# moritzmeister/hops-examples

Measured on AMD Instinct MI355X. Metric: images/sec MNIST CNN + steps/sec Chicago-taxi DNN at 1/2/4/8 MI355X, higher is better.
Workload: dtype bf16; 1 GPU; model=MNIST CNN (experiment.mirrored model, 1394282 params), Adadelta(1.0), global_batch=32, per_gpu_batch=32, parallelism=dp1, engine=PersistentMnistStep, hipgraph=False, steps_per_execution=32, warmup_steps_run=5

## Files before the change

csrc/ops/bindings.cpp:

```cpp
#include <pybind11/pybind11.h>
#include <pybind11/stl.h>

#include <algorithm>
#include <memory>
#include <stdexcept>
#include <string>
#include <tuple>
#include <utility>
#include <vector>

#if defined(HOPSX_DEBUG) && HOPSX_DEBUG
#define HOPSX_DEBUG_BUILD 1
#else
#define HOPSX_DEBUG_BUILD 0
#endif

#include "ops_api.h"
extern "C" int hopsx_mnist_persist_occupancy(int dp);
extern "C" void hopsx_mnist_persist_reload_knobs();
extern "C" int hopsx_pad_cin(const float* w, long R, int C, int cp, float* out, void* out16, hipStream_t st);
extern "C" int hopsx_unpad_cin_add(float* gpad, long R, int C, int cp, float* tgt, hipStream_t st);

namespace py = pybind11;
extern "C" void hopsx_mlp_head_debug(void* p);
// ... 106 lines not shown
  if (!e) e = hopsx_det_set_##tag(on);
    HOPSX_DET_TUS(X)
#undef X
    return e;
  });
  m.attr("DEBUG") = HOPSX_DEBUG_BUILD;
  m.def("dbg_read", []() {
    static const std::pair<const char*, int (*)(unsigned*)> tus[] = {
#define X(tag) {#tag, hopsx_dbg_read_##tag},
        HOPSX_DBG_TUS(X)
#undef X
    };
    std::vector<std::tuple<std::string, unsigned, unsigned, unsigned, unsigned>> out;
    for (const auto& t : tus) {
      unsigned v[4] = {0u, 0u, 0u, 0u};
      const int e = t.second(v);
      if (e) throw std::runtime_error(std::string("hopsx dbg_read: hip error ") + std::to_string(e));
      if (v[0]) out.emplace_back(t.first, v[0], v[1], v[2], v[3]);
    }
    return out;
  });
  m.def("det_lost", []() {
    unsigned n = 0;
#define X(tag) n += hopsx_det_lost_##tag();
    HOPSX_DET_TUS(X)
#undef X
    return n;
  });
  m.def("mnist_persist", [](std::vector<uint64_t> p, std::vector<long> iv, std::vector<float> fv, u st) {
    return hopsx_mnist_persist(p.data(), (int)p.size(), iv.data(), (int)iv.size(), fv.data(), (int)fv.size(),
                               S(st));
  });
  def_arg_slots<false>(m, "mnist_persist", [](const ArgSlots& a, hipStream_t st) {
    return hopsx_mnist_persist(a.p.data(), (int)a.p.size(), a.iv.data(), (int)a.iv.size(), a.fv.data(),
                               (int)a.fv.size(), st);
  });
  m.def("mnist_eval", [](std::vector<uint64_t> p, std::vector<long> iv, std::vector<float> fv, u st) {
    return hopsx_mnist_eval(p.data(), (int)p.size(), iv.data(), (int)iv.size(), fv.data(), (int)fv.size(), S(st));
  });
  m.def("mnist_eval_tile", []() { return hopsx_mnist_eval_tile(); });
  m.def("taxi_eval", [](std::vector<uint64_t> p, std::vector<long> iv, u st) {
    return hopsx_taxi_eval(p.data(), (int)p.size(), iv.data(), (int)iv.size(), S(st));
  });
  m.def("taxi_eval_bins", []() { return hopsx_taxi_eval_bins(); });
  m.def("mnist_persist_reload_knobs", []() { hopsx_mnist_persist_reload_knobs(); });
  m.def("mnist_persist_occupancy", [](int dp) { return hopsx_mnist_persist_occupancy(dp); });
  m.def("pad_cin", [](u w, long R, int C, int cp, u out, u out16, u st) {
    return hopsx_pad_cin(P<float>(w), R, C, cp, P<float>(out), P<void>(out16), S(st));
  });
  m.def("unpad_cin_add", [](u g, long R, int C, int cp, u tgt, u st) {
    return hopsx_unpad_cin_add(P<float>(g), R, C, cp, P<float>(tgt), S(st));
  });
  m.def("mnist_persist_geom", []() {
    std::vector<long> g(23);
    hopsx_mnist_persist_geom(g.data());
    return g;
  });
  m.def("widedeep_step", [](std::vector<uint64_t> p, std::vector<long> iv, std::vector<float> fv, u st) {
    return hopsx_widedeep_step(p.data(), (int)p.size(), iv.data(), (int)iv.size(), fv.data(), (int)fv.size(),
                               S(st));
  });
  m.def("conv2d_fwd_pool_ok", [](std::vector<int> g, int act, int pk) { return hopsx_conv_fwd_pool_ok(g.data(), act, pk); });
  m.def("conv2d_fwd_pool", [](u x, u w, std::vector<int> g, u out, u am, u bias, int act, float p, u rng,
                              unsigned salt, int pk, u st) {
    return hopsx_conv2d_fwd_pool(P<void>(x), P<void>(w), g.data(), P<void>(out), P<void>(am), P<float>(bias), act, p,
                                 P<unsigned long long>(rng), salt, pk, S(st));
  });
  m.def("conv2d_fwd_pool_in_ok", [](std::vector<int> g0, std::vector<int> g, int act) {
    return hopsx_conv_fwd_pool_in_ok(g0.data(), g.data(), act);
  });
  m.def("conv2d_fwd_pool_in", [](u x0, float xscale, float xshift, u w0, u b0, int act0, std::vector<int> g0, u y1,
                                 u w, std::vector<int> g, u out, u am, u bias, int act, float p, u rng, unsigned salt,
                                 u st) {
    return hopsx_conv2d_fwd_pool_in(P<void>(x0), xscale, xshift, P<void>(w0), P<float>(b0), act0, g0.data(),
                                    P<void>(y1), P<void>(w), g.data(), P<void>(out), P<void>(am), P<float>(bias), act,
                                    p, P<unsigned long long>(rng), salt, S(st));
  });
  m.def("conv2d_dgrad_fused_wgrad_ok", [](std::vector<int> g, std::vector<int> g0) {
    return hopsx_conv_dgrad_fused_wgrad_ok(g.data(), g0.data());
  });
  m.def("conv2d_dgrad_fused_wgrad", [](u dy, u w, std::vector<int> g, u yprev, int act, u colsum, u y, int yact,
                                       std::vector<int> g0, u x0, float xscale, float xshift, u dw0, u st) {
    return hopsx_conv2d_dgrad_mfma_ex(P<void>(dy), P<void>(w), g.data(), nullptr, P<void>(yprev), act,
                                      P<float>(colsum), P<void>(y), yact, g0.data(), P<void>(x0), xscale, xshift,
                                      P<float>(dw0), S(st));
  });
  m.def("wgrad_debug_times", [](int n) {
    std::vector<unsigned long long> v((size_t)n);
    hopsx_wgrad_debug_times(v.data(), n);
    return v;
  });
  m.def("head_ce_ok", [](int C, int KD) { return hopsx_head_ce_ok(C, KD); });
  m.def("head_ce", [](int kind, u logits, int lf32, u target, int B, int C, int KD, float gs, u h, u w, u dw, u db,
                      u dh, u loss, u correct, u bias, u lout, float dp, u drng, unsigned dsalt, u st) {
    return hopsx_head_ce(kind, P<void>(logits), lf32, P<void>(target), B, C, KD, gs, P<void>(h), P<void>(w),
                         P<float>(dw), P<float>(db), P<void>(dh), P<float>(loss), P<int>(correct), P<float>(bias),
                         P<void>(lout), dp, P<unsigned long long>(drng), dsalt, S(st));
  });
  m.def("mlp_head_lds", [](int C, int N1) { return hopsx_mlp_head_lds(C, N1); });
  m.def("mlp_head_debug", [](u p) { hopsx_mlp_head_debug(P<void>(p)); });
  m.def("graph_upload", [](u exec, u st) {
    return (int)hipGraphUpload(reinterpret_cast<hipGraphExec_t>(exec), S(st));
  });
  m.def("mlp_head", [](u x, u w1, u b1, int act1, u y, u ws, u arrive, int B, int K, int N1, int kind, u target,
                       int C, float gs, u w2, u b2, u dw2, u db2, u dh, u loss, u correct, u lout, int lf32, float dp,
                       u drng, unsigned dsalt, u st) {
    return hopsx_mlp_head(P<void>(x), P<void>(w1), P<float>(b1), act1, P<void>(y), P<float>(ws), P<unsigned>(arrive),
// ... 208 lines not shown
```

csrc/ops/mnist_persist.hip:

```cpp
#include "common.h"
#include "mnist_cnn.h"
#include "optim_core.h"
#include "wg_prims.h"

namespace mnistp {
using namespace wgp;
using namespace mnist_cnn;

constexpr int B = 32;
constexpr int NCONV = C2 * 128 + C2 + C1 * 4 + C1;
constexpr int OFF_B2 = C2 * 128, OFF_W1 = OFF_B2 + C2, OFF_B1 = OFF_W1 + C1 * 4;
constexpr int SLICE = 64, NSLICE = (NCONV + SLICE - 1) / SLICE;
constexpr int NRED = 19;
constexpr int NKC = (NPOS + NRED - 1) / NRED;
constexpr int NQ = SLICE / 4;
constexpr int NHEAD = B;
constexpr int GRID = NPOS + NHEAD;
constexpr int PAY = 272;
constexpr int PAY_DH = 0, PAY_H = 128, PAY_DL = 256, PAY_LOSS = 268, PAY_COR = 269;
constexpr int FL_A = 0, FL_B = 256, FL_C = 512, FL_D = 768, FL_WORDS = 1024;
constexpr int FL_EPOCH = FL_WORDS - 2;
constexpr int D_F32 = OFF_B2 * 2;
constexpr int D_BYTES = D_F32 + (NCONV - OFF_B2) * 4;
constexpr int TGB_N = NHEAD * (HID / 2);
constexpr int TG_WORDS = 2 * 2 * TGB_N;
static_assert(FL_WORDS % 2 == 0 && TGB_N % 256 == 0, "granules are 8-B aligned; every thread owns TGB_N / 256");

constexpr int DHS = row_stride(HID), DCS = row_stride(4 * B);
static_assert(DHS == 136 && DCS == 136, "strides the kernel was tuned with");

constexpr int L_W1 = 0;
constexpr int L_W2 = L_W1 + HID * W1S * 2;
constexpr int L_CW1 = L_W2 + C2 * W2S * 2;
constexpr int L_CB1 = L_CW1 + C1 * 4 * 4;
constexpr int L_CB2 = L_CB1 + C1 * 4;
constexpr int L_XIN = L_CB2 + C2 * 4;
constexpr int L_C1 = L_XIN + B * 16 * 4;
constexpr int L_POOL = L_C1 + B * 9 * C1S * 2;
constexpr int L_AM = L_POOL + B * PLS * 2;
constexpr int L_DH = L_AM + B * C2;
constexpr int L_DC2 = L_DH + B * DHS * 2;
constexpr int L_STG = L_DC2 + C2 * DCS * 2;
constexpr int L_RED = L_STG + NCONV * 4;
constexpr int L_SL = L_RED + NRED * SLICE * 4;
constexpr int L_KEEP = L_SL + 3 * 64 * 4;
constexpr int LDS_BYTES = L_KEEP + B * C2;

constexpr int H_W2 = 0;
constexpr int H_B2 = H_W2 + 3 * NCLS * HID * 4;
constexpr int H_B1 = H_B2 + 3 * 16 * 4;
constexpr int H_RED = H_B1 + 3 * HID * 4;
constexpr int H_H = H_RED + 8 * HID * 4;
constexpr int H_LOG = H_H + HID * 4;
constexpr int H_PAY = H_LOG + 16 * 4;
constexpr int H_ALL = H_PAY + PAY * 4;
constexpr int H_END = H_ALL + NHEAD * PAY * 4;
constexpr int H_DHS = H_END;
static_assert(H_DHS + B * DHS * 2 <= LDS_BYTES, "head LDS map must fit the position map");

constexpr int XMAX = 8;
constexpr long XS_POOL = (long)NPOS * 4 * 64 * 16;
constexpr long XS_DHT = 8L * 64 * 16;
constexpr int NFC2 = NCLS * HID + HID + NCLS, NFC2P = 1424;
constexpr long XS_FC2 = NFC2P * 4;
constexpr long XS_CONV = (long)NSLICE * SLICE * 4;
constexpr long XO_POOL = 0, XO_DHT = XO_POOL + 2L * XMAX * XS_POOL, XO_FC2 = XO_DHT + 2L * XMAX * XS_DHT,
               XO_CONV = XO_FC2 + 2L * XMAX * XS_FC2, X_BYTES = XO_CONV + 2L * XMAX * XS_CONV;
constexpr int XF_POOL = 0, XF_H = XMAX * NPOS, XF_CONV = XF_H + XMAX, XF_WORDS = XF_CONV + XMAX * NSLICE;
static_assert(NFC2 <= NFC2P && NFC2P % 4 == 0 && X_BYTES < 0x7fffffffL, "exchange geometry");
static_assert(LDS_BYTES <= 160 * 1024, "one workgroup per CU: 160 KiB LDS");
static_assert(L_RED + NRED * SLICE * 4 <= L_SL && 2 * 32 * 5 * 4 <= NRED * SLICE * 4, "reduce scratch");
static_assert(SLICE * 4 % 128 == 0 && NCONV * 4 % 128 == 0, "a slice row is whole 128-byte lines of an aligned slabC row");
static_assert(OFF_B2 % SLICE == 0 && D_F32 % 128 == 0 && D_BYTES % 128 == 0, "no slice straddles the bf16 / fp32 parts of D");
static_assert(NSLICE * SLICE >= NCONV && NSLICE <= NPOS && SLICE == 64, "slice geometry: one wave updates a slice");
static_assert(NQ == 16 && NRED > 16 && NRED - 16 <= 3 && 5 * NKC <= 64 && 2 * NKC <= 32 && NRED * (NKC - 1) < NPOS,
              "gather geometry: at most 5 groups' flags per wave, one per lane; both items' rows in one pend mask");

struct Args {
  float* master;
// ... 196 lines not shown
      if (__builtin_amdgcn_readfirstlane(e) != 0u) {
        good = 0;
        break;
      }
      if ((spins & 15u) == 15u && wall_clock64() - t0 > tmo) {
        if (lane == 0) atomicCAS(err, 0u, code);
        good = 0;
        break;
      }
      __builtin_amdgcn_s_sleep(1);
    }
    if (lane == 0) *s_ok = good;
  }
  __syncthreads();
  const int v = *s_ok;
  return v != 0;
}
template <int N, class F>
__device__ __forceinline__ bool sweep_tags(const unsigned long long* g, int tid, unsigned epoch, unsigned* err,
                                        unsigned code, int* s_fail, long long tmo, F put) {
  unsigned pend = (1u << N) - 1u;
  unsigned long long x[N];
#pragma unroll
  for (int k = 0; k < N; ++k) x[k] = granule_load(g + tid + 256 * k);
  unsigned e = flag_load(err);
  const long long t0 = wall_clock64();
  for (unsigned spins = 0;; ++spins) {
#pragma unroll
    for (int k = 0; k < N; ++k)
      if (((pend >> k) & 1u) && (unsigned)(x[k] >> 32) == epoch) {
        put(tid + 256 * k, (unsigned)x[k]);
        pend &= ~(1u << k);
      }
    if (!__any(pend != 0u)) break;
    bool bad = __builtin_amdgcn_readfirstlane(e) != 0u;
    if (!bad && (spins & 15u) == 15u && wall_clock64() - t0 > tmo) {
      if ((threadIdx.x & 63) == 0) atomicCAS(err, 0u, code);
      bad = true;
    }
    if (bad) {
      if ((threadIdx.x & 63) == 0) *s_fail = 1;
      break;
    }
#pragma unroll
    for (int k = 0; k < N; ++k)
      if ((pend >> k) & 1u) x[k] = granule_load(g + tid + 256 * k);
    e = flag_load(err);
  }
  __syncthreads();
  const int f = *s_fail;
  return f == 0;
}

template <int NK, class L>
__device__ __forceinline__ void gather_rows(const unsigned* flag, bool mine, int shift, unsigned pend, unsigned epoch,
                                            unsigned* err, unsigned code, int* s_fail, long long tmo, L load) {
  const long long t0 = wall_clock64();
  for (unsigned spins = 0;; ++spins) {
    const unsigned e = flag_load(err);
    const unsigned f = mine ? flag_load(flag) : 0u;
    const unsigned long long here = __ballot(mine && f == epoch);
    const unsigned now = pend & (unsigned)(here >> shift);
#pragma unroll
    for (int k = 0; k < NK; ++k)
      if ((now >> k) & 1u) load(k);
    pend &= ~now;
    if (!__any(pend != 0u)) break;
    bool bad = __builtin_amdgcn_readfirstlane(e) != 0u;
    if (!bad && (spins & 15u) == 15u && wall_clock64() - t0 > tmo) {
      if ((threadIdx.x & 63) == 0) atomicCAS(err, 0u, code);
      bad = true;
    }
    if (bad) {
      if ((threadIdx.x & 63) == 0) *s_fail = 1;
      break;
    }
    __builtin_amdgcn_s_sleep(1);
  }
}

template <bool DP>
__device__ __forceinline__ void position_wg(const Args& a, unsigned char* smem, int* s_ok, const OptHP& hp,
                                            long long cur0, unsigned long long seed, unsigned long long ctr0,
                                            long long xs0, unsigned long long eb) {
  const int p = blockIdx.x, ph = p / PH, pw = p - ph * PH;
  const int tid = threadIdx.x, lane = tid & 63, w = tid >> 6, fr = lane & 15, fq = lane >> 4;
  const int tq = fr >> 2, tp = fr & 3;
  bf16_raw* W1 = (bf16_raw*)(smem + L_W1);
  bf16_raw* W2 = (bf16_raw*)(smem + L_W2);
  float* CW1 = (float*)(smem + L_CW1);
  float* CB1 = (float*)(smem + L_CB1);
  float* CB2 = (float*)(smem + L_CB2);
  float* XIN = (float*)(smem + L_XIN);
  bf16_raw* C1 = (bf16_raw*)(smem + L_C1);
  bf16_raw* POOL = (bf16_raw*)(smem + L_POOL);
  unsigned char* AM = smem + L_AM;
  bf16_raw* DH = (bf16_raw*)(smem + L_DH);
  bf16_raw* DC2 = (bf16_raw*)(smem + L_DC2);
  float* STG = (float*)(smem + L_STG);
  float* RED = (float*)(smem + L_RED);
  float* SLm = (float*)(smem + L_SL);
  float* SL1 = SLm + 64;
  float* SL2 = SLm + 128;

  float wm[2][4][4], g1[2][4][4], g2[2][4][4];
#pragma unroll
  for (int ii = 0; ii < 2; ++ii)
#pragma unroll
    for (int j = 0; j < 4; ++j)
#pragma unroll
      for (int r = 0; r < 4; ++r) {
        const int n = (2 * w + ii) * 16 + fq * 4 + r, co = j * 16 + fr;
        const long ai = a.off[4] + (long)n * KIN + p * C2 + co;
        wm[ii][j][r] = a.master[ai];
        g1[ii][j][r] = a.s1[ai];
        g2[ii][j][r] = a.s2[ai];
        W1[n * W1S + co] = f2bf_hw(wm[ii][j][r]);
      }
  auto put_conv = [&](int j, float v) {
    if (j < OFF_B2) W2[(j >> 7) * W2S + (j & 127)] = f2bf_hw(v);
    else if (j < OFF_W1) CB2[j - OFF_B2] = v;
    else if (j < OFF_B1) CW1[j - OFF_W1] = v;
    else CB1[j - OFF_B1] = v;
  };
  {
    constexpr int NJ = (NCONV + 255) / 256;
    float cv[NJ];
#pragma unroll
    for (int q = 0; q < NJ; ++q) {
      const int j = tid + 256 * q;
// ... 151 lines not shown
    stamp(a, s, 1);
    {
      f32x4 acc[2][2];
#pragma unroll
      for (int i = 0; i < 2; ++i)
#pragma unroll
        for (int jj = 0; jj < 2; ++jj) acc[i][jj] = (f32x4){0.f, 0.f, 0.f, 0.f};
      bf16x8 af[2][2], bfr[2][2];
#pragma unroll
      for (int kk = 0; kk < 2; ++kk) {
#pragma unroll
        for (int i = 0; i < 2; ++i) af[kk][i] = lds8(POOL + (i * 16 + fr) * PLS + kk * 32 + fq * 8);
#pragma unroll
        for (int jj = 0; jj < 2; ++jj) bfr[kk][jj] = lds8(W1 + ((2 * w + jj) * 16 + fr) * W1S + kk * 32 + fq * 8);
      }
      __builtin_amdgcn_sched_barrier(0);
#pragma unroll
      for (int kk = 0; kk < 2; ++kk)
#pragma unroll
        for (int i = 0; i < 2; ++i)
#pragma unroll
          for (int jj = 0; jj < 2; ++jj) acc[i][jj] = mma32(af[kk][i], bfr[kk][jj], acc[i][jj]);
#pragma unroll
      for (int i = 0; i < 2; ++i)
#pragma unroll
        for (int jj = 0; jj < 2; ++jj)
#pragma unroll
          for (int r = 0; r < 4; ++r) STG[(i * 16 + fq * 4 + r) * HID + (2 * w + jj) * 16 + fr] = acc[i][jj][r];
    }
    __syncthreads();
    {
      const auto R = rsrc(a.slabA + ((long)par * NPOS + p) * (B * HID));
      f32x4 v[4];
#pragma unroll
      for (int k = 0; k < 4; ++k) v[k] = *(const f32x4*)(STG + (tid + 256 * k) * 4);
      __builtin_amdgcn_sched_barrier(0);
#pragma unroll
      for (int k = 0; k < 4; ++k) bst16<SC1>(R, (tid + 256 * k) * 16, v[k]);
      drain();
      __syncthreads();
      if (tid == 0) flag_store(a.flags + FL_A + p, ep);
    }
    const unsigned gep = (unsigned)(xs0 + s + 1);
    if constexpr (DP) {
      const int c0 = w * 16 + 4 * tp;
      const f32x4 f = __builtin_bit_cast(f32x4, lds_tr(POOL + (8 * fq + tq) * PLS + c0, POOL + (8 * fq + tq + 4) * PLS + c0));
      for (int r = 0; r < a.world; ++r) {
        if (r == a.rank) continue;
        bst16<SYS>(rsrc(a.xbuf[r] + XO_POOL + (par * XMAX + xslot(a, r)) * XS_POOL + (long)p * 4096), (w * 64 + lane) * 16, f);
      }
    }
    if (s + 1 < a.nsteps) xv = xload(s + 1);
    stamp(a, s, 2);
    if (a.hand & 1) {
      const unsigned long long* TB = (const unsigned long long*)(a.flags + FL_WORDS) + par * TGB_N;
      const unsigned code = s ? ecode(2, s) : ecode(12, 0);
      const long long tmo = s ? a.tmo : a.tmo0;
      if (!gate_tags(TB, p & (HID / 2 - 1), ep, (a.hand >> 8), a.err, code, s_ok, tmo)) return;
      if (!sweep_tags<TGB_N / 256>(TB, tid, ep, a.err, code, s_ok + 2, tmo, [&](int idx, unsigned v) {
            *(unsigned*)(DH + (idx >> 6) * DHS + 2 * (idx & 63)) = v;
          }))
        return;
      if constexpr (DP) {
        drain();
        __syncthreads();
        if (tid < 64) raise_peers(a, XF_POOL + p, NPOS, gep);
      }
      stamp(a, s, 3);
    } else {
    if (!wait_all(a.flags + FL_B, NHEAD, ep, a.err, s ? ecode(2, s) : ecode(12, 0), a.acquire, s_ok,
                  s ? a.tmo : a.tmo0, a.pollw_b, a.stagger, (a.hand & 2)))
      return;
    if constexpr (DP) {
      drain();
      __syncthreads();
      if (tid < 64) raise_peers(a, XF_POOL + p, NPOS, gep);
    }
    stamp(a, s, 3);
    {
      const auto R = rsrc(a.slabB + (long)par * NHEAD * PAY);
#pragma unroll
      for (int k = 0; k < 4; ++k) {
        const int idx = tid + 256 * k, b = idx >> 5, n4 = idx & 31;
        const f32x4 v = bld16<SC1>(R, (b * PAY + PAY_DH + n4 * 4) * 4);
        *(bf16x4*)(DH + b * DHS + n4 * 4) =
            (bf16x4){(short)f2bf_hw(v[0]), (short)f2bf_hw(v[1]), (short)f2bf_hw(v[2]), (short)f2bf_hw(v[3])};
      }
    }
    __syncthreads();
    }
    f32x4 gw[2][4], dp[2];
    unsigned char amv[2][4];
    {
      bf16x8 da[4][2], db4[4];
#pragma unroll
      for (int kk = 0; kk < 4; ++kk) {
        const int k1 = kk * 32 + 8 * fq + tq;
        db4[kk] = lds_tr(W1 + k1 * W1S + w * 16 + 4 * tp, W1 + (k1 + 4) * W1S + w * 16 + 4 * tp);
#pragma unroll
        for (int i = 0; i < 2; ++i) da[kk][i] = lds8(DH + (i * 16 + fr) * DHS + kk * 32 + fq * 8);
      }
#pragma unroll
      for (int i = 0; i < 2; ++i)
#pragma unroll
        for (int r = 0; r < 4; ++r) amv[i][r] = AM[(i * 16 + fq * 4 + r) * C2 + w * 16 + fr];
      __builtin_amdgcn_sched_barrier(0);
      dp[0] = dp[1] = (f32x4){0.f, 0.f, 0.f, 0.f};
#pragma unroll
      for (int kk = 0; kk < 4; ++kk)
#pragma unroll
        for (int i = 0; i < 2; ++i) dp[i] = mma32(da[kk][i], db4[kk], dp[i]);
    }
    {
      const int co = w * 16 + fr;
      float db = 0.f;
#pragma unroll
      for (int i = 0; i < 2; ++i)
#pragma unroll
        for (int r = 0; r < 4; ++r) {
          const int b = i * 16 + fq * 4 + r;
          const int am = amv[i][r];
          const bf16_raw gb = am != 0xFF ? f2bf_hw(dp[i][r] * inv) : (bf16_raw)0;
          db += bf2f(gb);
          *(bf16x4*)(DC2 + co * DCS + b * 4) = (bf16x4){(short)(am == 0 ? gb : 0), (short)(am == 1 ? gb : 0),
                                                        (short)(am == 2 ? gb : 0), (short)(am == 3 ? gb : 0)};
        }
      db += __shfl_xor(db, 16, 64);
      db += __shfl_xor(db, 32, 64);
      if (fq == 0) STG[OFF_B2 + co] = db;
    }
    {
      f32x4 acc[8];
#pragma unroll
      for (int j = 0; j < 8; ++j) acc[j] = (f32x4){0.f, 0.f, 0.f, 0.f};
      const bf16_raw* cb = C1 + (2 * fq * 9 + (tq >> 1) * 3 + (tq & 1)) * C1S + 4 * tp;
      bf16x8 af[2], bfr[2][8];
      auto cfrag = [&](int kk, int st) {
#pragma unroll
        for (int j = 0; j < 8; ++j) {
          const int t = j >> 1;
          const bf16_raw* q = cb + (kk * 8 * 9 + (t >> 1) * 3 + (t & 1)) * C1S + (j & 1) * 16;
          bfr[st][j] = lds_tr(q, q + 9 * C1S);
        }
      };
// ... 105 lines not shown
            gk[0] = fmaf(dd, xi[py][px], gk[0]);
            gk[1] = fmaf(dd, xi[py][px + 1], gk[1]);
            gk[2] = fmaf(dd, xi[py + 1][px], gk[2]);
            gk[3] = fmaf(dd, xi[py + 1][px + 1], gk[3]);
            gk[4] += dd;
          }
      }
#pragma unroll
      for (int k = 0; k < 5; ++k) {
        gk[k] += __shfl_xor(gk[k], 16, 64);
        gk[k] += __shfl_xor(gk[k], 32, 64);
      }
      if (fq == 0) {
#pragma unroll
        for (int k = 0; k < 5; ++k) RED[(mh * 32 + ci) * 5 + k] = gk[k];
      }
    }
    __syncthreads();
    if (tid < 32 * 5) {
      const int ci = tid / 5, k = tid - ci * 5;
      const float v = RED[ci * 5 + k] + RED[(32 + ci) * 5 + k];
      if (k < 4) STG[OFF_W1 + ci * 4 + k] = v;
      else STG[OFF_B1 + ci] = v;
    }
    __syncthreads();
    stamp(a, s, 5);
    {
      const auto R = rsrc(a.slabC + ((long)par * NPOS + p) * NCONV);
      const int idx = OFF_B2 / 4 + tid;
      if (idx < NCONV / 4) bst16<SC1>(R, idx * 16, *(const f32x4*)(STG + idx * 4));
      drain();
      __syncthreads();
      if (tid == 0) flag_store(a.flags + FL_C + p, ep);
    }
    stamp(a, s, 6);
    if (owner) {
      const int e0 = p * SLICE;
      const int j = lane & (NQ - 1), lq = lane >> 4, g = 4 * w + lq, gx = 16 + w;
      const bool act = e0 + 4 * j < NCONV, two = lq == 3 && gx < NRED;
      const auto R = rsrc(a.slabC + (long)par * NPOS * NCONV);
      f32x4 v[2 * NKC];
#pragma unroll
      for (int k = 0; k < 2 * NKC; ++k) v[k] = (f32x4){0.f, 0.f, 0.f, 0.f};
      auto load = [&](int k) {
        const int pp = k < NKC ? g + NRED * k : gx + NRED * (k - NKC);
        v[k] = bld16<SC1>(R, (pp * NCONV + e0 + 4 * j) * 4);
      };
      const unsigned rows2 = gx + NRED * (NKC - 1) < NPOS ? (1u << NKC) - 1u : (1u << (NKC - 1)) - 1u;
      const unsigned pend = !act ? 0u : ((1u << NKC) - 1u) | (two ? rows2 << NKC : 0u);
      bool lost = false;
      if ((a.hand & 8) && !a.acquire) {
        const int lp = lane < 4 * NKC ? 4 * w + lane / NKC + NRED * (lane % NKC) : gx + NRED * (lane - 4 * NKC);
        const bool mine = lane < 4 * NKC || (gx < NRED && lane < 5 * NKC && lp < NPOS);
        gather_rows<2 * NKC>(a.flags + FL_C + lp, mine, lq * NKC, pend, ep, a.err, ecode(3, s), s_ok + 2, a.tmo, load);
        stamp(a, s, 7);
      } else {
        lost = !wait_all(a.flags + FL_C, NPOS, ep, a.err, ecode(3, s), a.acquire, s_ok, a.tmo, a.pollw_c, a.stagger,
                         (a.hand & 2));
        stamp(a, s, 7);
#pragma unroll
        for (int k = 0; k < 2 * NKC; ++k)
          if (!lost && ((pend >> k) & 1u)) load(k);
      }
#pragma unroll
      for (int k = 0; k < 2 * NKC; ++k) asm volatile("" ::"v"(v[k]));
      {
        f32x4 acc = (f32x4){0.f, 0.f, 0.f, 0.f};
#pragma unroll
        for (int k = 0; k < NKC; ++k) acc += v[k];
        *(f32x4*)(RED + g * SLICE + 4 * j) = acc;
      }
      if (two) {
        f32x4 acc = (f32x4){0.f, 0.f, 0.f, 0.f};
#pragma unroll
        for (int k = 0; k < NKC; ++k) acc += v[NKC + k];
        *(f32x4*)(RED + gx * SLICE + 4 * j) = acc;
      }
      __syncthreads();
      {
        const int f = s_ok[2];
        if (lost || f) return;
      }
      const int e = e0 + tid;
      float gs = 0.f;
      if (tid < SLICE) {
        for (int g = 0; g < NRED; ++g) gs += RED[g * SLICE + tid];
      }
      if constexpr (DP) {
        if (tid < 64) {
          if (tid < SLICE) {
            for (int r = 0; r < a.world; ++r) {
              if (r == a.rank) continue;
              bst4<SYS>(rsrc(a.xbuf[r] + XO_CONV + (par * XMAX + xslot(a, r)) * XS_CONV), e * 4, gs);
            }
          }
          drain();
          raise_peers(a, XF_CONV + p, NSLICE, gep);
        }
        if (!wait_peers(a, XF_CONV + p, NSLICE, gep, ecode(6, s), s_ok)) return;
        if (tid < SLICE) {
          const auto X = rsrc(a.xbuf[a.rank] + XO_CONV + (long)par * XMAX * XS_CONV);
          float v[XMAX];
#pragma unroll
          for (int r = 0; r < XMAX; ++r) v[r] = r < a.world && r != a.rank ? bld4<SYS>(X, (int)(r * XS_CONV) + e * 4) : gs;
          float t = 0.f;
#pragma unroll
          for (int r = 0; r < XMAX; ++r)
// ... 20 lines not shown
        drain();
        if (lane == 0) flag_store(a.flags + FL_D + p, ep);
      }
      stamp(a, s, 8);
    }
    if constexpr (DP) {
      if (!wait_peers(a, XF_H, 1, gep, ecode(7, s), s_ok)) return;
      if (!wait_peers(a, XF_POOL + p, NPOS, gep, ecode(8, s), s_ok)) return;
#pragma unroll
      for (int ii = 0; ii < 2; ++ii)
#pragma unroll
        for (int j = 0; j < 4; ++j) gw[ii][j] = (f32x4){0.f, 0.f, 0.f, 0.f};
      const auto XP = rsrc(a.xbuf[a.rank] + XO_POOL + (long)par * XMAX * XS_POOL + (long)p * 4096);
      const auto XD = rsrc(a.xbuf[a.rank] + XO_DHT + (long)par * XMAX * XS_DHT);
      constexpr int PF = 3;
      bf16x8 af[PF][2], bfr[PF][4];
      auto fetch = [&](int r, int b) {
        if (r == a.rank) {
#pragma unroll
          for (int ii = 0; ii < 2; ++ii) {
            const int n0 = (2 * w + ii) * 16 + 4 * tp;
            af[b][ii] = lds_tr(DH + (8 * fq + tq) * DHS + n0, DH + (8 * fq + tq + 4) * DHS + n0);
          }
#pragma unroll
          for (int j = 0; j < 4; ++j) {
            const int c0 = j * 16 + 4 * tp;
            bfr[b][j] = lds_tr(POOL + (8 * fq + tq) * PLS + c0, POOL + (8 * fq + tq + 4) * PLS + c0);
          }
        } else {
#pragma unroll
          for (int ii = 0; ii < 2; ++ii)
            af[b][ii] = __builtin_bit_cast(bf16x8, bld16<SYS>(XD, (int)(r * XS_DHT) + ((2 * w + ii) * 64 + lane) * 16));
#pragma unroll
          for (int j = 0; j < 4; ++j)
            bfr[b][j] = __builtin_bit_cast(bf16x8, bld16<SYS>(XP, (int)(r * XS_POOL) + (j * 64 + lane) * 16));
        }
      };
#pragma unroll
      for (int r = 0; r < PF - 1; ++r)
        if (r < a.world) fetch(r, r);
#pragma unroll
      for (int r = 0; r < XMAX; ++r) {
        if (r < a.world) {
          if (r + PF - 1 < XMAX && r + PF - 1 < a.world) fetch(r + PF - 1, (r + PF - 1) % PF);
#pragma unroll
          for (int ii = 0; ii < 2; ++ii)
#pragma unroll
            for (int j = 0; j < 4; ++j)
              gw[ii][j] += mma32(af[r % PF][ii], bfr[r % PF][j], (f32x4){0.f, 0.f, 0.f, 0.f});
        }
      }
    }
#pragma unroll
    for (int ii = 0; ii < 2; ++ii)
#pragma unroll
      for (int j = 0; j < 4; ++j)
#pragma unroll
        for (int r = 0; r < 4; ++r) {
          wm[ii][j][r] = adadelta(wm[ii][j][r], gw[ii][j][r] * hp.gscale, g1[ii][j][r], g2[ii][j][r], hp);
          W1[((2 * w + ii) * 16 + fq * 4 + r) * W1S + j * 16 + fr] = f2bf_hw(wm[ii][j][r]);
        }
    if (s + 1 < a.nsteps) draw_keep(s + 1);
    stamp(a, s, 9);
    if (!owner && tid < 64) {
      constexpr int G0 = OFF_B2 / SLICE;
      const bool mine = lane < NSLICE - G0;
      const long long t0 = wall_clock64();
      for (;;) {
        const unsigned f = mine ? flag_load(a.flags + FL_D + G0 + lane) : ep;
        if (__all(f == ep) || wall_clock64() - t0 > 2000) break;
        __builtin_amdgcn_s_sleep(4);
      }
    }
    if (!wait_all(a.flags + FL_D, NSLICE, ep, a.err, ecode(4, s), a.acquire, s_ok, a.tmo, a.pollw_d, a.stagger,
                  (a.hand & 2)))
      return;
    stamp(a, s, 10);
    {
      const auto R = rsrc((const unsigned char*)a.slabD + (long)par * D_BYTES);
      constexpr int NB = OFF_B2 * 2 / 16;
      constexpr int NF = (NCONV - OFF_B2) / 4;
      f32x4 dv[NB / 256 + 1];
#pragma unroll
      for (int k = 0; k < NB / 256; ++k) dv[k] = bld16<SC1>(R, (tid + 256 * k) * 16);
      dv[NB / 256] = tid < NF ? bld16<SC1>(R, D_F32 + tid * 16) : (f32x4){0.f, 0.f, 0.f, 0.f};
#pragma unroll
      for (int k = 0; k < NB / 256; ++k) {
        const int c = tid + 256 * k;
        *(f32x4*)(W2 + (c >> 4) * W2S + (c & 15) * 8) = dv[k];
      }
      if (tid < NF) {
        const int j = OFF_B2 + tid * 4;
        float* dst = j < OFF_W1 ? CB2 + (j - OFF_B2) : (j < OFF_B1 ? CW1 + (j - OFF_W1) : CB1 + (j - OFF_B1));
        *(f32x4*)dst = dv[NB / 256];
      }
    }
    __syncthreads();
    stamp(a, s, 11);
  }

#pragma unroll
  for (int ii = 0; ii < 2; ++ii)
#pragma unroll
    for (int j = 0; j < 4; ++j)
#pragma unroll
      for (int r = 0; r < 4; ++r) {
        const int n = (2 * w + ii) * 16 + fq * 4 + r, co = j * 16 + fr;
        const long ai = a.off[4] + (long)n * KIN + p * C2 + co;
        a.master[ai] = wm[ii][j][r];
        a.s1[ai] = g1[ii][j][r];
        a.s2[ai] = g2[ii][j][r];
        a.shadow[ai] = f2bf_hw(wm[ii][j][r]);
      }
  if (owner && tid < SLICE) {
    const int e = p * SLICE + tid;
// ... 349 lines not shown
  if (blockIdx.x < NPOS) {
    position_wg<DP>(a, smem, s_ok, hp, cur0, a.rng[0], a.rng[1], xs0, eb);
  } else {
    head_wg<DP>(a, smem, s_ok, hp, cur0, xs0, eb);
  }
}

}

static int g_persist_reload = 0;
extern "C" void hopsx_mnist_persist_reload_knobs() { g_persist_reload = 1; }

extern "C" int hopsx_mnist_persist(const uint64_t* p, int np, const long* iv, int ni, const float* fv, int nf,
                                   hipStream_t st) {
  using namespace mnistp;
  if (np < 18 || ni < 18 || nf < 8) return (int)hipErrorInvalidValue;
  if (iv[11] != B || iv[10] < 1 || iv[8] < 1) return (int)hipErrorInvalidValue;
  const int world = (int)iv[13], rank = (int)iv[14];
  if (world < 1 || world > XMAX || rank < 0 || rank >= world) return (int)hipErrorInvalidValue;
  const bool dp = world > 1;
  if (dp && np < 19 + 2 * world) return (int)hipErrorInvalidValue;
  Args a{};
  a.master = (float*)p[0];
  a.shadow = (bf16_raw*)p[1];
  a.s1 = (float*)p[2];
  a.s2 = (float*)p[3];
  a.xs = (const unsigned char*)p[4];
  a.ys = (const long long*)p[5];
  a.cursor = (long long*)p[6];
  a.rng = (unsigned long long*)p[7];
  a.step_dev = (float*)p[8];
  a.hp_dev = (const float*)p[9];
  a.slabA = (float*)p[10];
  a.slabB = (float*)p[11];
  a.slabC = (float*)p[12];
  a.slabD = (float*)p[13];
  a.flags = (unsigned*)p[14];
  a.err = (unsigned*)p[15];
  a.out = (float*)p[16];
  a.dbg = (unsigned long long*)p[17];
  if (((uint64_t)a.slabC & 127) || ((uint64_t)a.slabD & 127)) return (int)hipErrorInvalidValue;
  for (int k = 0; k < 8; ++k) a.off[k] = iv[k];
  a.nbatch = iv[8];
  a.salt = (unsigned)iv[9];
  a.nsteps = (int)iv[10];
  a.acquire = (int)iv[12];
  a.world = world;
  a.rank = rank;
  a.loopback = (int)iv[15];
  a.xfence = (int)iv[17];
  a.tmo = (long long)iv[16] * 100000ll;
  a.tmo0 = a.tmo;
  static int kn_ok = 0, kn_pollw, kn_stagger, kn_a, kn_b, kn_c, kn_d, kn_head1w, kn_memset, kn_coop;
  static int kn_tagged, kn_gate, kn_poll1, kn_prog;
  static long kn_start_ms;
  if (!kn_ok || g_persist_reload) {
    auto pw = [&](const char* name, long dflt) {
      const long v = hopsx_env_int(name, dflt);
      return (int)(v >= 1 && v <= 4 ? v : 1);
    };
    kn_pollw = pw("HOPSX_PERSIST_POLLW", 1);
    kn_stagger = (int)hopsx_env_int("HOPSX_PERSIST_STAGGER", 12);
    kn_a = pw("HOPSX_PERSIST_POLLW_A", kn_pollw);
    kn_b = pw("HOPSX_PERSIST_POLLW_B", kn_pollw);
    kn_c = pw("HOPSX_PERSIST_POLLW_C", 4);
    kn_d = pw("HOPSX_PERSIST_POLLW_D", kn_pollw);
    kn_head1w = (int)hopsx_env_int("HOPSX_PERSIST_HEAD1W", 1);
    kn_memset = (int)hopsx_env_int("HOPSX_PERSIST_MEMSET", 0);
    kn_coop = (int)hopsx_env_int("HOPSX_PERSIST_COOP", 0);
    kn_start_ms = hopsx_env_int("HOPSX_PERSIST_START_MS", 50);
    kn_tagged = hopsx_env_int("HOPSX_PERSIST_TAGGED", 1) != 0;
    const long gt = hopsx_env_int("HOPSX_PERSIST_GATE", NHEAD / 2);
    kn_gate = (int)(gt >= 1 && gt <= NHEAD ? gt : NHEAD / 2);
    kn_poll1 = hopsx_env_int("HOPSX_PERSIST_POLL1", 1) != 0;
    kn_prog = (int)(hopsx_env_int("HOPSX_PERSIST_PROG", 3) & 2);
    kn_ok = 1;
    g_persist_reload = 0;
  }
  a.pollw = kn_pollw;
  a.stagger = kn_stagger;
  a.pollw_a = kn_a;
  a.pollw_b = kn_b;
  a.pollw_c = kn_c;
  a.pollw_d = kn_d;
  a.head1w = kn_head1w;
  a.hand = kn_tagged | (kn_poll1 << 1) | (kn_prog << 2) | (kn_gate << 8);
  if (kn_start_ms > 0 && kn_start_ms * 100000ll < a.tmo) a.tmo0 = kn_start_ms * 100000ll;
  a.inv_gb = 1.f / (float)(world * B);
  if (dp) {
    a.xstep = (long long*)p[18];
    for (int r = 0; r < world; ++r) {
      a.xbuf[r] = (unsigned char*)p[19 + r];
      a.xflag[r] = (unsigned*)p[19 + world + r];
      if (!a.xbuf[r] || !a.xflag[r] || ((uint64_t)a.xbuf[r] & 15)) return (int)hipErrorInvalidValue;
    }
  }
  a.drop_p = fv[0];
  a.xscale = fv[1];
  a.xshift = fv[2];
  a.hp = OptHP{fv[3], fv[4], fv[5], fv[6], fv[7], 0.f, 0.f, 0.f};
  static bool attr[2] = {false, false};
  const void* fn = dp ? (const void*)mnist_persist_k<true> : (const void*)mnist_persist_k<false>;
  if (!attr[dp]) {
    const hipError_t e = hipFuncSetAttribute(fn, hipFuncAttributeMaxDynamicSharedMemorySize, LDS_BYTES);
    if (e != hipSuccess) return (int)e;
    attr[dp] = true;
  }
  if (kn_memset) {
    const hipError_t e = hipMemsetAsync(a.flags, 0, FL_WORDS * sizeof(unsigned), st);
    if (e != hipSuccess) return (int)e;
  }
  if (kn_coop) {
    void* kargs[] = {(void*)&a};
    const hipError_t e = hipLaunchCooperativeKernel(fn, dim3(GRID), dim3(256), kargs, LDS_BYTES, st);
    if (e != hipSuccess) {
      (void)hipGetLastError();
      return (int)e;
    }
    return (int)hipSuccess;
  }
  if (dp)
    hipLaunchKernelGGL(mnist_persist_k<true>, dim3(GRID), dim3(256), LDS_BYTES, st, a);
  else
    hipLaunchKernelGGL(mnist_persist_k<false>, dim3(GRID), dim3(256), LDS_BYTES, st, a);
  return (int)hipGetLastError();
}

extern "C" int hopsx_mnist_persist_occupancy(int dp) {
  using namespace mnistp;
  const void* fn = dp ? (const void*)mnist_persist_k<true> : (const void*)mnist_persist_k<false>;
  if (hipFuncSetAttribute(fn, hipFuncAttributeMaxDynamicSharedMemorySize, LDS_BYTES) != hipSuccess) return -1;
  int n = 0;
  if (hipOccupancyMaxActiveBlocksPerMultiprocessor(&n, fn, 256, LDS_BYTES) != hipSuccess) return -1;
  return n;
}

extern "C" void hopsx_mnist_persist_geom(long* g) {
  using namespace mnistp;
  g[0] = B;
  g[1] = NPOS;
  g[2] = NHEAD;
  g[3] = GRID;
  g[4] = NCONV;
  g[5] = NSLICE;
  g[6] = SLICE;
  g[7] = PAY;
  g[8] = FL_WORDS;
  g[9] = LDS_BYTES;
  g[10] = D_BYTES;
  g[11] = X_BYTES;
  g[12] = XF_WORDS;
  g[13] = XMAX;
  g[14] = XO_POOL;
  g[15] = XS_POOL;
  g[16] = XO_DHT;
  g[17] = XS_DHT;
  g[18] = XO_FC2;
  g[19] = XS_FC2;
  g[20] = XO_CONV;
  g[21] = XS_CONV;
  g[22] = TG_WORDS;
}
```

hops_examples_amd/runtime/persist.py:

```python
from __future__ import annotations

import os

import torch

from .launch_slots import ArgSlots, launch_shapes

_GEOM = None


def _ext():
    from ..ops import _C

    return _C.ext()


def geometry() -> dict:
    global _GEOM
    if _GEOM is None:
        g = _ext().mnist_persist_geom()
        _GEOM = dict(zip(["batch", "npos", "nhead", "grid", "nconv", "nslice", "slice", "pay", "flag_words",
                          "lds_bytes", "d_bytes", "x_bytes", "xflag_words", "max_ranks", "xo_pool", "xs_pool",
                          "xo_dht", "xs_dht", "xo_fc2", "xs_fc2", "xo_conv", "xs_conv", "tag_words"], g))
    return _GEOM


class PersistentError(RuntimeError):
    pass


def flagship_layers(model):
    from .. import nn as hnn
    from ..models.mnist import MirroredMnistCNN

    names = ("conv1", "conv2", "pool", "fc1", "fc2")
    L = [getattr(model, n, None) for n in names]
    if any(x is None for x in L):
        return None
    c1, c2, pool, f1, f2 = L

    def conv_ok(c, cin, cout):
        return (isinstance(c, hnn.Conv2d) and c.in_channels == cin and c.out_channels == cout
                and tuple(c.kernel_size) == (2, 2) and c.activation == "relu" and c.bias is not None
                and c.cfg.get("stride", 1) in (1, (1, 1)) and c.cfg.get("padding", 0) in (0, "valid", (0, 0))
                and c.cfg.get("dilation", 1) in (1, (1, 1)))

    def dense_ok(d, fin, fout, act):
        return (isinstance(d, hnn.Linear) and tuple(d.weight.shape) == (fout, fin) and d.activation == act
                and d.bias is not None)

    ok = (conv_ok(c1, 1, 32) and conv_ok(c2, 32, 64) and c1.in_affine is not None
          and isinstance(pool, hnn.MaxPool2d) and pool.k == 2 and pool.s in (None, 2) and not pool.p
          and 0.0 <= float(pool.dropout) < 1.0
          and dense_ok(f1, 13 * 13 * 64, 128, "relu") and dense_ok(f2, 128, 10, None))
    return L if ok and type(model).forward is MirroredMnistCNN.forward else None


def _device_cus(dev) -> int:
    return int(torch.cuda.get_device_properties(dev).multi_processor_count)


def _occupancy(dp: bool) -> int:
    return int(_ext().mnist_persist_occupancy(int(dp)))


def launchable(dev, world: int = 1) -> tuple[bool, str]:
    g = geometry()
    cus = _device_cus(dev)
    if cus < g["grid"]:
        return False, f"{cus} CUs < the persistent grid of {g['grid']} workgroups"
    occ = _occupancy(world > 1)
    if occ < 1:
        return False, f"occupancy {occ} workgroups per CU"
    return True, "ok"


# ... 476 lines not shown
```

Measured before the change: 1.463 million images/sec.

## Fill spin-wait in row gather with chunked fc1 Adadelta updates and early keep-mask draw

```diff
diff --git a/csrc/ops/bindings.cpp b/csrc/ops/bindings.cpp
--- a/csrc/ops/bindings.cpp
+++ b/csrc/ops/bindings.cpp
@@ -182,7 +182,7 @@
     return hopsx_unpad_cin_add(P<float>(g), R, C, cp, P<float>(tgt), S(st));
   });
   m.def("mnist_persist_geom", []() {
-    std::vector<long> g(23);
+    std::vector<long> g(24);
     hopsx_mnist_persist_geom(g.data());
     return g;
   });
diff --git a/csrc/ops/mnist_persist.hip b/csrc/ops/mnist_persist.hip
--- a/csrc/ops/mnist_persist.hip
+++ b/csrc/ops/mnist_persist.hip
@@ -25,6 +25,11 @@
 constexpr int TGB_N = NHEAD * (HID / 2);
 constexpr int TG_WORDS = 2 * 2 * TGB_N;
 static_assert(FL_WORDS % 2 == 0 && TGB_N % 256 == 0, "granules are 8-B aligned; every thread owns TGB_N / 256");
+constexpr int HAND_FILL_C = 1 << 16;
+constexpr int HAND_FILL_KEEP = 1 << 17;
+constexpr int HAND_FMAX_SHIFT = 20;
+constexpr int FCH = 4, NFCH = 32 / FCH;
+static_assert(32 % FCH == 0 && NFCH <= 15, "whole chunks; the cap fits its 4 bits of Args::hand");
 
 constexpr int DHS = row_stride(HID), DCS = row_stride(4 * B);
 static_assert(DHS == 136 && DCS == 136, "strides the kernel was tuned with");
@@ -327,13 +332,16 @@
   return f == 0;
 }
 
-template <int NK, class L>
+template <int NK, class L, class F>
 __device__ __forceinline__ void gather_rows(const unsigned* flag, bool mine, int shift, unsigned pend, unsigned epoch,
-                                            unsigned* err, unsigned code, int* s_fail, long long tmo, L load) {
+                                            unsigned* err, unsigned code, int* s_fail, long long tmo, L load, F fill) {
   const long long t0 = wall_clock64();
   for (unsigned spins = 0;; ++spins) {
     const unsigned e = flag_load(err);
     const unsigned f = mine ? flag_load(flag) : 0u;
+    __builtin_amdgcn_sched_barrier(0);
+    const bool filled = fill();
+    __builtin_amdgcn_sched_barrier(0);
     const unsigned long long here = __ballot(mine && f == epoch);
     const unsigned now = pend & (unsigned)(here >> shift);
 #pragma unroll
@@ -350,7 +358,7 @@
       if ((threadIdx.x & 63) == 0) *s_fail = 1;
       break;
     }
-    __builtin_amdgcn_s_sleep(1);
+    if (!filled) __builtin_amdgcn_s_sleep(1);
   }
 }
 
@@ -608,11 +616,12 @@
     }
     if (s + 1 < a.nsteps) xv = xload(s + 1);
     stamp(a, s, 2);
+    if ((a.hand & HAND_FILL_KEEP) && s + 1 < a.nsteps) draw_keep(s + 1);
     if (a.hand & 1) {
       const unsigned long long* TB = (const unsigned long long*)(a.flags + FL_WORDS) + par * TGB_N;
       const unsigned code = s ? ecode(2, s) : ecode(12, 0);
       const long long tmo = s ? a.tmo : a.tmo0;
-      if (!gate_tags(TB, p & (HID / 2 - 1), ep, (a.hand >> 8), a.err, code, s_ok, tmo)) return;
+      if (!gate_tags(TB, p & (HID / 2 - 1), ep, (a.hand >> 8) & 0xFF, a.err, code, s_ok, tmo)) return;
       if (!sweep_tags<TGB_N / 256>(TB, tid, ep, a.err, code, s_ok + 2, tmo, [&](int idx, unsigned v) {
             *(unsigned*)(DH + (idx >> 6) * DHS + 2 * (idx & 63)) = v;
           }))
@@ -646,6 +655,15 @@
     __syncthreads();
     }
     f32x4 gw[2][4], dp[2];
+    auto fc1_chunk = [&](int c) {
+#pragma unroll
+      for (int q = 0; q < FCH; ++q) {
+        const int el = c * FCH + q, ii = el >> 4, j = (el >> 2) & 3, r = el & 3;
+        wm[ii][j][r] = adadelta(wm[ii][j][r], gw[ii][j][r] * hp.gscale, g1[ii][j][r], g2[ii][j][r], hp);
+        W1[((2 * w + ii) * 16 + fq * 4 + r) * W1S + j * 16 + fr] = f2bf_hw(wm[ii][j][r]);
+      }
+    };
+    unsigned fleft = (1u << NFCH) - 1u;
     unsigned char amv[2][4];
     {
       bf16x8 da[4][2], db4[4];
@@ -857,7 +875,19 @@
       if ((a.hand & 8) && !a.acquire) {
         const int lp = lane < 4 * NKC ? 4 * w + lane / NKC + NRED * (lane % NKC) : gx + NRED * (lane - 4 * NKC);
         const bool mine = lane < 4 * NKC || (gx < NRED && lane < 5 * NKC && lp < NPOS);
-        gather_rows<2 * NKC>(a.flags + FL_C + lp, mine, lq * NKC, pend, ep, a.err, ecode(3, s), s_ok + 2, a.tmo, load);
+        int fcap = !DP && (a.hand & HAND_FILL_C) ? (a.hand >> HAND_FMAX_SHIFT) & 15 : 0;
+        auto fill = [&]() -> bool {
+          if (fcap <= 0) return false;
+          const unsigned bit = __builtin_amdgcn_readfirstlane(fleft & (0u - fleft));
+#pragma unroll
+          for (int c = 0; c < NFCH; ++c)
+            if ((bit >> c) & 1u) fc1_chunk(c);
+          fleft &= ~bit;
+          --fcap;
+          return true;
+        };
+        gather_rows<2 * NKC>(a.flags + FL_C + lp, mine, lq * NKC, pend, ep, a.err, ecode(3, s), s_ok + 2, a.tmo, load,
+                             fill);
         stamp(a, s, 7);
       } else {
         lost = !wait_all(a.flags + FL_C, NPOS, ep, a.err, ecode(3, s), a.acquire, s_ok, a.tmo, a.pollw_c, a.stagger,
@@ -984,15 +1014,9 @@
       }
     }
 #pragma unroll
-    for (int ii = 0; ii < 2; ++ii)
-#pragma unroll
-      for (int j = 0; j < 4; ++j)
-#pragma unroll
-        for (int r = 0; r < 4; ++r) {
-          wm[ii][j][r] = adadelta(wm[ii][j][r], gw[ii][j][r] * hp.gscale, g1[ii][j][r], g2[ii][j][r], hp);
-          W1[((2 * w + ii) * 16 + fq * 4 + r) * W1S + j * 16 + fr] = f2bf_hw(wm[ii][j][r]);
-        }
-    if (s + 1 < a.nsteps) draw_keep(s + 1);
+    for (int c = 0; c < NFCH; ++c)
+      if ((__builtin_amdgcn_readfirstlane(fleft) >> c) & 1u) fc1_chunk(c);
+    if (!(a.hand & HAND_FILL_KEEP) && s + 1 < a.nsteps) draw_keep(s + 1);
     stamp(a, s, 9);
     if (!owner && tid < 64) {
       constexpr int G0 = OFF_B2 / SLICE;
@@ -1448,7 +1472,7 @@
   a.tmo = (long long)iv[16] * 100000ll;
   a.tmo0 = a.tmo;
   static int kn_ok = 0, kn_pollw, kn_stagger, kn_a, kn_b, kn_c, kn_d, kn_head1w, kn_memset, kn_coop;
-  static int kn_tagged, kn_gate, kn_poll1, kn_prog;
+  static int kn_tagged, kn_gate, kn_poll1, kn_prog, kn_fill, kn_fmax;
   static long kn_start_ms;
   if (!kn_ok || g_persist_reload) {
     auto pw = [&](const char* name, long dflt) {
@@ -1470,6 +1494,9 @@
     kn_gate = (int)(gt >= 1 && gt <= NHEAD ? gt : NHEAD / 2);
     kn_poll1 = hopsx_env_int("HOPSX_PERSIST_POLL1", 1) != 0;
     kn_prog = (int)(hopsx_env_int("HOPSX_PERSIST_PROG", 3) & 2);
+    kn_fill = (int)(hopsx_env_int("HOPSX_PERSIST_FILL", 3) & 3);
+    const long fm = hopsx_env_int("HOPSX_PERSIST_FILL_MAX", NFCH);
+    kn_fmax = (int)(fm >= 0 && fm <= NFCH ? fm : NFCH);
     kn_ok = 1;
     g_persist_reload = 0;
   }
@@ -1480,7 +1507,7 @@
   a.pollw_c = kn_c;
   a.pollw_d = kn_d;
   a.head1w = kn_head1w;
-  a.hand = kn_tagged | (kn_poll1 << 1) | (kn_prog << 2) | (kn_gate << 8);
+  a.hand = kn_tagged | (kn_poll1 << 1) | (kn_prog << 2) | (kn_gate << 8) | (kn_fill << 16) | (kn_fmax << HAND_FMAX_SHIFT);
   if (kn_start_ms > 0 && kn_start_ms * 100000ll < a.tmo) a.tmo0 = kn_start_ms * 100000ll;
   a.inv_gb = 1.f / (float)(world * B);
   if (dp) {
@@ -1556,4 +1583,5 @@
   g[20] = XO_CONV;
   g[21] = XS_CONV;
   g[22] = TG_WORDS;
-}
+  g[23] = NFCH;
+}
diff --git a/hops_examples_amd/runtime/persist.py b/hops_examples_amd/runtime/persist.py
--- a/hops_examples_amd/runtime/persist.py
+++ b/hops_examples_amd/runtime/persist.py
@@ -21,7 +21,8 @@
         g = _ext().mnist_persist_geom()
         _GEOM = dict(zip(["batch", "npos", "nhead", "grid", "nconv", "nslice", "slice", "pay", "flag_words",
                           "lds_bytes", "d_bytes", "x_bytes", "xflag_words", "max_ranks", "xo_pool", "xs_pool",
-                          "xo_dht", "xs_dht", "xo_fc2", "xs_fc2", "xo_conv", "xs_conv", "tag_words"], g))
+                          "xo_dht", "xs_dht", "xo_fc2", "xs_fc2", "xo_conv", "xs_conv", "tag_words", "fill_chunks"],
+                         g))
     return _GEOM
 
 
```

New measurement: 1.523 million images/sec, median of 6. +4.1%, better.
